# SayanoAI/Comfy-RVC

Measured on AMD Instinct MI355X. Metric: audio-sec/wall-sec (xRT), 40k_v2 end-to-end VC, higher is better.
Workload: dtype f32; 1 GPU; Full VC 40k_v2 (HuBERT -> RMVPE -> SynthesizerTrnMs768NSFsid), 30 s 16 kHz clips, 12 per GPU per step (3 in flight), vc_single host array in -> int16 host array out (BASELINE.json configs[2]); clips_in_flight_per_gpu=3, weights=procedural (comfy-rvc_amd/synthetic.py), noise=device generator, seeded per clip, parallelism=clip-per-GPU x1 (3 lanes each), one RCCL gather of the step's int16 waveforms

## Files before the change

### comfy-rvc_amd/_lib.py

```python
import ctypes as C
import os

_HERE = os.path.dirname(os.path.abspath(__file__))
LIB_PATH = os.environ.get("RVC_HIP_LIB") or os.path.join(_HERE, "csrc", "librvc_hip.so")


class RvcHipError(RuntimeError):
    pass


def _load():
    if not os.path.isfile(LIB_PATH):
        raise RvcHipError(
            f"{LIB_PATH} is missing: build it with `python -c 'import __graft_entry__ as g; g.build()'` "
            "(or `make -C comfy-rvc_amd/csrc`).  There is no CPU fallback.")
    return C.CDLL(LIB_PATH)


lib = _load()

c_void_p, c_int, c_int64, c_float, c_char_p = C.c_void_p, C.c_int, C.c_int64, C.c_float, C.c_char_p
P = C.POINTER


# ... 140 lines not shown
    "rvc_declick": (c_int, [c_void_p, c_void_p, c_int64, c_int, c_float, c_int, c_int, c_int, c_void_p, c_void_p]),
    "rvc_peak_normalize": (c_int, [c_void_p, c_void_p, c_int64, c_float, c_void_p]),
    "rvc_peak_limit": (c_int, [c_void_p, c_void_p, c_int64, c_float]),
    "rvc_merge_tracks": (c_int, [c_void_p, P(c_void_p), P(c_int64), c_int, c_int, c_void_p, c_int64]),
    "rvc_segment_energy": (c_int, [c_void_p, c_void_p, c_int64, c_int, c_void_p]),
    "rvc_spectrogram_batch": (c_int, [c_void_p, c_void_p, c_void_p, c_int64, c_void_p, c_int, c_int, c_int, c_float, c_int, c_void_p, c_int64]),
    "rvc_mel_filterbank_set": (c_int, [c_void_p, c_int, c_int, c_void_p, c_void_p, c_void_p]),
    "rvc_spec_to_mel_batch": (c_int, [c_void_p, c_void_p, c_void_p, c_int64, c_void_p, c_int, c_int, c_int, c_void_p, c_int64]),
    "rvc_spectrogram_batch_ms": (c_int, [c_void_p, c_void_p, c_void_p, c_int64, c_void_p, c_int, c_int, c_int, c_float, c_int, c_void_p, c_int64]),
    "rvc_multiscale_mel_loss": (c_int, [c_void_p, c_void_p, c_int, P(c_void_p), P(c_int64), P(c_int64), c_int, c_int64, P(C.c_int32), P(C.c_int32), c_int, c_int,
                                        c_void_p]),
    "rvc_hpss": (c_int, [c_void_p, c_void_p, c_int, c_int, c_int, c_void_p, c_void_p, c_int]),
    "rvc_hpss_l1": (c_int, [c_void_p, c_void_p, c_void_p, c_int, c_int, c_int, c_float, c_void_p]),
    "rvc_tsi_terms": (c_int, [c_void_p, c_void_p, c_void_p, c_int, c_int, c_int, c_float, c_void_p]),
    "rvc_op_gemm_split": (c_int, [c_void_p] * 7 + [c_int] * 4 + [c_float, c_int, c_float] + [c_int] * 5),
    "rvc_op_conv2d_split": (c_int, [c_void_p] * 7 + [c_int] * 9),
    "rvc_op_wn_in_gate_split": (c_int, [c_void_p] * 6 + [c_int] * 4),
    "rvc_op_gemm_split_qkv": (c_int, [c_void_p] * 6 + [c_int] * 4),
    "rvc_op_conv1d_s2_split": (c_int, [c_void_p] * 6 + [c_int] * 5),
    "rvc_op_conv1d_split": (c_int, [c_void_p] * 6 + [c_int] * 9),
    "rvc_op_conv1d": (c_int, [c_void_p, c_void_p, c_void_p, c_void_p, c_void_p, c_void_p] + [c_int] * 8 +
                      [c_int, c_float, c_int, c_float, c_int, c_float, c_int]),
    "rvc_op_conv_transpose1d": (c_int, [c_void_p, c_void_p, c_void_p, c_void_p, c_void_p] + [c_int] * 6 + [c_int, c_float, c_int]),
    "rvc_op_conv2d3x3": (c_int, [c_void_p, c_void_p, c_void_p, c_void_p, c_void_p, c_void_p] + [c_int] * 5),
    "rvc_op_conv_transpose2d": (c_int, [c_void_p, c_void_p, c_void_p, c_void_p, c_void_p] + [c_int] * 5),
    "rvc_op_gemm_tn": (c_int, [c_void_p, c_void_p, c_void_p, c_void_p] + [c_int] * 4),
    "rvc_conv1d_plan_create": (c_int, [c_void_p, c_void_p] + [c_int] * 7 + [P(c_void_p)]),
    "rvc_conv1d_plan_run": (c_int, [c_void_p, c_void_p, c_void_p, c_int, c_void_p, c_void_p, c_int, c_float, c_int, c_float]),
    "rvc_conv1d_plan_pair_run": (c_int, [c_void_p, c_void_p, c_void_p, c_void_p, c_int, c_void_p, c_float, c_int]),
    "rvc_conv1d_plan_resblock_run": (c_int, [P(c_void_p), c_void_p, c_void_p, c_int, c_void_p, c_float, c_int, P(c_int), c_void_p, c_void_p, c_void_p]),
# ... 108 lines not shown
```

### comfy-rvc_amd/csrc/conv_x3s.hip

```cpp
#include "conv_x3_dev.h"
#include "ops.h"

namespace rvc {

struct GemmSArgs {
  const unsigned char* Wx; int CoPx;
  const unsigned char* Xs; long long xsTp;
  unsigned wx_bytes, xs_bytes;
  int Co, T, nunits;
  int ktaps, margin;
  int toff[16];
  int groups, co_g, rows_pg, cig_chunks;
  unsigned wg_bytes;
  int tdil, tpad;
  int padw; unsigned padmagic;
  const float* bias; const float* R; long long ldR;
  float* Y; long long ldY;
  unsigned char* Ys; long long ysTp;
  int act; float act_slope; int act_before_res; float out_scale;
  int ksplit; float* slabs; unsigned* tickets;
  int gx, gy;
  int xcd_remap;
  int ymargin;
  int zero_tail;
  int row_fast;
  unsigned char* Vt; long long vtTp;
  int vt_row0, vt_rows;
  const float* gate_g; int gate_h;
  int ydeint;
  int seg2_u, seg2_soff;
};

RVC_PHASE_TABLE_REGISTER;

constexpr int x3s_wgs(int AM, int AN, int RS) { return (AM * AN >= 4 && RS != 3) ? 2 : 3; }
template <int AM, int AN, int RS>
__global__ __launch_bounds__(256, x3s_wgs(AM, AN, RS)) void conv_x3s_kernel(const GemmSArgs p) {
  constexpr int WN = 2, NW = 4;
  constexpr int BM = 64 * AM, BN = 64 * AN;
  constexpr int NPA = BM / 16, NPB = BN / 16, NPW = (NPA + NPB) / NW;
  static_assert((NPA % NW) == 0 && (NPB % NW) == 0, "every wave's i-th piece is of one kind");
  constexpr int aslot = BM * 64, bslot = BN * 64, uslot = aslot + bslot;
  static_assert(RS >= 3 && (RS - 2) * NPW <= 63, "ring");
  extern __shared__ __attribute__((aligned(1024))) unsigned char smem3s[];

  const int tid0 = threadIdx.x;
  int lane = tid0 & 63;
  const int wave = __builtin_amdgcn_readfirstlane(tid0 >> 6);
  const int wm = wave / WN, wn = wave % WN;
  const int li = lane & 31, lh = lane >> 5;
  const unsigned total = gridDim.x;
  const unsigned bid = p.xcd_remap ? xcd_tile(blockIdx.x, total) : blockIdx.x;
  const int S = p.ksplit;
  const int tile = (int)(bid / (unsigned)S), ks = (int)(bid - (unsigned)tile * (unsigned)S);
  const int tile_y = p.row_fast ? tile % p.gy : tile / p.gx, tile_x = p.row_fast ? tile / p.gy : tile - tile_y * p.gx;
  const int grp = tile_y / p.rows_pg;
  const int co0 = (tile_y - grp * p.rows_pg) * BM, n0 = tile_x * BN;
  const int row0 = grp * p.co_g, CoG = p.co_g;
// ... 14 lines not shown
#pragma unroll
        for (int an = 0; an < AN; ++an) {
          const int n = n0 + (wn * AN + an) * 32 + li;
          acc[am][an][r] = buf_load(rrs, (r_pre && m < CoG && n < p.T) ? ((unsigned)(row0 + m) * (unsigned)p.ldR + (unsigned)n) * 4u : kOOB) + bv;
        }
      }
  } else {
#pragma unroll
    for (int am = 0; am < AM; ++am)
#pragma unroll
      for (int an = 0; an < AN; ++an)
#pragma unroll
        for (int r = 0; r < 16; ++r) acc[am][an][r] = 0.f;
  }

  const __amdgpu_buffer_rsrc_t ars = make_rsrc(p.Wx, p.wx_bytes), brs = make_rsrc(p.Xs, p.xs_bytes);
  int voff[NPW], dsto[NPW];
#pragma unroll
  for (int i = 0; i < NPW; ++i) {
    const int pi = wave + NW * i;
    if (i * NW < NPA) {
      constexpr int RBK = BM / 64;
      const int plane = pi / RBK, rb = pi - plane * RBK;
      voff[i] = (plane * p.CoPx + co0 + rb * 64 + lane) * 16;
      dsto[i] = plane * (BM * 16) + rb * 1024;
    } else {
      constexpr int CBK = BN / 64;
      const int pj = pi - NPA, plane = pj / CBK, cb = pj - plane * CBK;
      voff[i] = (int)((plane * p.xsTp + n0 + cb * 64 + lane) * 16);
      dsto[i] = aslot + plane * (BN * 16) + cb * 1024;
    }
  }
  const int KT = p.ktaps;
  const int wstep = p.CoPx * 64, cstep = (int)(p.xsTp * 64);
  int tap = u0 % KT;
  bool seg2 = false;
  const bool arith = KT > 16;
  auto tap_off = [&](int t) { return arith ? t * p.tdil - p.tpad : p.toff[t & 15]; };
  int soff_a = (int)((unsigned)grp * p.wg_bytes) + u0 * wstep, soff_c = (grp * p.cig_chunks + u0 / KT) * cstep, soff_b = soff_c + (p.margin + tap_off(tap)) * 16;
  if (u0 >= p.seg2_u) { seg2 = true; soff_b = p.seg2_soff + (u0 - p.seg2_u) * cstep + p.margin * 16; }
  const int seg2_at = p.seg2_u - u0;
  int slw = 0, uw = 0;
  auto issue = [&]() {
    unsigned char* base = smem3s + slw * uslot;
#pragma unroll
    for (int i = 0; i < NPW; ++i) {
      if (i * NW < NPA) buf_dma(ars, base + dsto[i], voff[i], soff_a);
      else buf_dma(brs, base + dsto[i], voff[i], soff_b);
    }
    ++uw;
    if (uw < U1) {
      soff_a += wstep;
      if (uw == seg2_at) { seg2 = true; soff_b = p.seg2_soff + p.margin * 16; }
      else if (KT > 1 && !seg2) {
        ++tap;
        if (tap == KT) { tap = 0; soff_c += cstep; }
        soff_b = soff_c + (p.margin + tap_off(tap)) * 16;
      } else {
        soff_b += cstep;
      }
    }
    slw = slw + 1 == RS ? 0 : slw + 1;
  };

  const int aoff = lh * (BM * 16) + ((wm * AM) * 32 + li) * 16;
  const int boff = aslot + lh * (BN * 16) + ((wn * AN) * 32 + li) * 16;

#pragma unroll
  for (int i = 0; i < RS - 1; ++i) issue();
  wait_vmcnt<(RS - 2) * NPW>();
#pragma unroll
  for (int am = 0; am < AM; ++am)
#pragma unroll
    for (int an = 0; an < AN; ++an) asm volatile("" : "+v"(acc[am][an]));
  lds_barrier();

  struct Ops { u32x4 ah[AM], al[AM], bh[AN], bl[AN]; };
  Ops o0, o1;
  auto read_ops = [&](Ops& o, int slot_i) {
    const unsigned char* wa = smem3s + slot_i * uslot + aoff;
    const unsigned char* xa = smem3s + slot_i * uslot + boff;
#pragma unroll
    for (int am = 0; am < AM; ++am) { o.ah[am] = *reinterpret_cast<const u32x4*>(wa + am * 512); o.al[am] = *reinterpret_cast<const u32x4*>(wa + BM * 32 + am * 512); }
#pragma unroll
    for (int an = 0; an < AN; ++an) { o.bh[an] = *reinterpret_cast<const u32x4*>(xa + an * 512); o.bl[an] = *reinterpret_cast<const u32x4*>(xa + BN * 32 + an * 512); }
  };
  auto mfmas = [&](const Ops& o) {
#pragma unroll
    for (int am = 0; am < AM; ++am)
#pragma unroll
      for (int an = 0; an < AN; ++an)
        acc[am][an] = __builtin_amdgcn_mfma_f32_32x32x16_bf16(__builtin_bit_cast(bf16x8, o.ah[am]), __builtin_bit_cast(bf16x8, o.bl[an]), acc[am][an], 0, 0, 0);
#pragma unroll
    for (int am = 0; am < AM; ++am)
#pragma unroll
      for (int an = 0; an < AN; ++an)
        acc[am][an] = __builtin_amdgcn_mfma_f32_32x32x16_bf16(__builtin_bit_cast(bf16x8, o.al[am]), __builtin_bit_cast(bf16x8, o.bh[an]), acc[am][an], 0, 0, 0);
#pragma unroll
    for (int am = 0; am < AM; ++am)
#pragma unroll
      for (int an = 0; an < AN; ++an)
        acc[am][an] = __builtin_amdgcn_mfma_f32_32x32x16_bf16(__builtin_bit_cast(bf16x8, o.ah[am]), __builtin_bit_cast(bf16x8, o.bh[an]), acc[am][an], 0, 0, 0);
  };
  int sl = 0;
  auto body = [&](const Ops& cur, Ops& nxt) {
    tm.lap(2);
    wait_vmcnt<(RS - 3) * NPW>();
    tm.lap(3);
    lds_barrier();
    tm.lap(4);
    issue();
    sl = sl + 1 == RS ? 0 : sl + 1;
    read_ops(nxt, sl);
    __builtin_amdgcn_sched_barrier(0);
    mfmas(cur);
    __builtin_amdgcn_sched_barrier(0);
  };
  read_ops(o0, 0);
  tm.lap(1);
  int u = 0;
  for (; u + 1 < U1; u += 2) { body(o0, o1); body(o1, o0); }
  if (u < U1) body(o0, o1);
  tm.lap(2);
  asm volatile("s_waitcnt vmcnt(0)" ::: "memory");
  tm.mark();

  if (S > 1) {
    typedef float f32x4_t __attribute__((ext_vector_type(4)));
    constexpr int QN = AM * AN * 4;
    const unsigned slab_bytes = 256u * QN * 16u;
    const __amdgpu_buffer_rsrc_t srs = make_rsrc(p.slabs, (unsigned)(total) * slab_bytes);
    const unsigned lane_off = ((unsigned)wave * QN * 64u + (unsigned)lane) * 16u;
    {
      const unsigned mine = ((unsigned)tile * (unsigned)S + (unsigned)ks) * slab_bytes + lane_off;
#pragma unroll
      for (int am = 0; am < AM; ++am)
#pragma unroll
        for (int an = 0; an < AN; ++an)
#pragma unroll
          for (int q = 0; q < 4; ++q) {
// ... 320 lines not shown
    const int c = hp * 8 + 2 * j;
    if (c < C) Y[(long long)c * ldY + t] = __uint_as_float(hi[j] << 16) + __uint_as_float(lo[j] << 16);
    if (c + 1 < C) Y[(long long)(c + 1) * ldY + t] = __uint_as_float(hi[j] & 0xffff0000u) + __uint_as_float(lo[j] & 0xffff0000u);
  }
}
void split_image_deint_from_f32(hipStream_t s, const float* X, long long ldX, int C, int T, unsigned char* img, long long tp, int H) {
  hipLaunchKernelGGL(split_image_deint_kernel, dim3((T + 255) / 256, (C + 15) / 16 * 2), dim3(256), 0, s, X, ldX, C, T, img, tp, H);
}
void split_image_deint_to_f32(hipStream_t s, const unsigned char* img, long long tp, int H, int C, int T, float* Y, long long ldY) {
  hipLaunchKernelGGL(unsplit_image_deint_kernel, dim3((T + 255) / 256, (C + 15) / 16 * 2), dim3(256), 0, s, img, tp, H, C, T, Y, ldY);
}
void split_image_to_f32(hipStream_t s, const unsigned char* img, long long tp, int C, int T, float* Y, long long ldY) {
  hipLaunchKernelGGL(unsplit_image_kernel, dim3((T + 255) / 256, (C + 15) / 16 * 2), dim3(256), 0, s, img, tp, C, T, Y, ldY);
}

template <int AM, int AN, int RS>
static void launch_x3s(const GemmSArgs& a, unsigned blocks, hipStream_t s) {
  auto kern = conv_x3s_kernel<AM, AN, RS>;
  constexpr size_t lds = (size_t)RS * (64 * AM + 64 * AN) * 64;
  RVC_ALLOW_BIG_LDS(kern);
  conv_launch(kern, dim3(blocks), dim3(256), lds, s, a);
}
static void x3s_dispatch(const GemmSArgs& a, int AM, int AN, unsigned blocks, hipStream_t s) {
  const bool rs3 = AM == 2 && AN == 2 && blocks >= 768u && a.nunits / a.ksplit >= 64;
  if (AM == 2 && AN == 2) { if (rs3) launch_x3s<2, 2, 3>(a, blocks, s); else launch_x3s<2, 2, 4>(a, blocks, s); }
  else if (AM == 2 && AN == 1) launch_x3s<2, 1, 4>(a, blocks, s);
  else if (AM == 1 && AN == 2) launch_x3s<1, 2, 4>(a, blocks, s);
  else launch_x3s<1, 1, 4>(a, blocks, s);
}

static thread_local int t_force_s = 0, t_force_am = 0, t_force_an = 0;
void conv_x3s_force(int ksplit, int am, int an) { t_force_s = ksplit; t_force_am = am; t_force_an = an; }
static void x3s_plan(int M, long long Nplan, int units, int& AM, int& AN, int& S, int groups = 1) {
  static const int target = exp_int("RVC_X3S_BLK", 440);
  auto tiles = [&](int am, int an) { return (long long)groups * ((M + 64 * am - 1) / (64 * am)) * ((Nplan + 64 * an - 1) / (64 * an)); };
  AM = 2; AN = 2;
  const bool deep = units >= 128 && groups == 1 && tiles(2, 2) >= 256;
  if (!deep && tiles(AM, AN) < target) AN = 1;
  if (!deep && tiles(AM, AN) < target) AM = 1;
  if (groups > 1) AM = 1;
  if ((t_force_am == 1 || t_force_am == 2) && groups == 1) AM = t_force_am;
  if (t_force_an == 1 || t_force_an == 2) AN = t_force_an;
  S = 1;
  const long long nt = tiles(AM, AN);
  static const int min_units = exp_int("RVC_X3S_MINUNITS", 32);
  for (int c : {2, 3, 4, 6, 8, 12, 16}) {
    if (nt * S >= target) break;
    if (units % c == 0 && units / c >= min_units) S = c;
  }
  if (t_force_s > 0) S = (units % t_force_s == 0 && units / t_force_s >= 4) ? t_force_s : 1;
}

bool conv_x3s_eligible(const ConvLayer& L) {
  if (L.Wx_ == nullptr || (L.Ci & 15) != 0 || L.Ci * L.ktaps < 32 || L.tconv_u != 0 || L.up2 != 0) return false;
  if (L.mode == 2) return L.ktaps <= 16;
  if (L.mode != 1 || L.stride != 1 || L.pad > kSplitMargin || (L.k - 1) * L.dil - L.pad > kSplitMargin) return false;
  if (L.groups > 1) return (L.Co & 15) == 0 && (L.CoPx & 63) == 0 && L.CoPx <= 64;
  return L.k <= 16 && L.pad == (L.k - 1) / 2 * L.dil && (L.k & 1) == 1;
}

SplitGeom split_geom_s2(int k, long long Tin) {
  SplitGeom g; g.ktaps = k; g.s2_h = split_s2_h(Tin); g.margin = kSplitMargin; g.padw = 0;
  RVC_REQUIRE(k >= 1 && k <= 16, "split_geom_s2: at most 16 taps");
  for (int t = 0; t < k; ++t) g.toff[t] = (t & 1) * g.s2_h + (t >> 1);
  return g;
// ... 59 lines not shown
    a.gate_h = e.gate_h; a.gate_g = e.gate_g;
  }
  a.vt_row0 = 0x7fffffff;
  if (e.vt_out) {
    RVC_REQUIRE(G == 1 && L.mode == 1 && e.vt_row0 > 0 && (e.vt_row0 & 127) == 0 && e.vt_row0 < L.Co && e.vt_tp >= kSplitMargin + (L.Co - e.vt_row0) && Y == nullptr && !e.R && !s2,
                "conv_x3s_run: the transposed rows are the tail of an image-only k = 1 projection, from a multiple of 128 rows on");
    a.Vt = e.vt_out; a.vtTp = e.vt_tp; a.vt_row0 = e.vt_row0; a.vt_rows = L.Co - e.vt_row0;
  }
  a.padmagic = geom->padw > 0 ? (unsigned)((0x100000000ULL + (unsigned)geom->padw - 1) / (unsigned)geom->padw) : 0u;
  for (int t = 0; t < 16; ++t) a.toff[t] = t < geom->ktaps ? geom->toff[t] : 0;
  a.tdil = L.mode == 1 ? L.dil : 1; a.tpad = L.mode == 1 ? L.pad : 0;
  if (s2) { a.tdil = 1; a.tpad = 0; }
  a.groups = G; a.co_g = L.Co; a.cig_chunks = L.Ci / 16; a.wg_bytes = (unsigned)((double)(L.Ci / 16) * geom->ktaps * 4.0 * (double)L.CoPx * 16.0);
  a.bias = e.bias_override ? e.bias_override : L.bd_; a.R = e.R; a.ldR = e.ldR; a.Y = Y; a.ldY = ldY; a.Ys = e.ys_out; a.ysTp = e.ys_tp;
  a.act = e.act; a.act_slope = e.act_slope; a.act_before_res = e.act_before_res; a.out_scale = e.out_scale;
  int AM, AN, S;
  x3s_plan(L.Co, e.plan_tin > 0 ? e.plan_tin : T, a.nunits, AM, AN, S, G);
  const int BM = 64 * AM, BN = 64 * AN;
  RVC_REQUIRE(L.CoPx % BM == 0, "weight image rows are padded to the tile");
  a.rows_pg = (L.Co + BM - 1) / BM;
  a.gx = (T + BN - 1) / BN; a.gy = a.rows_pg * G; a.ksplit = S;
  a.xcd_remap = x3_xcd_remap();
  const unsigned blocks = (unsigned)((long long)a.gx * a.gy * S);
  if (S > 1) {
    const size_t slab_bytes = (size_t)blocks * BM * BN * 4;
    const size_t tick_bytes = ((size_t)a.gx * a.gy * 4 + 255) & ~(size_t)255;
    static const size_t kTickCap = 64 * 1024;
    RVC_REQUIRE(tick_bytes <= kTickCap, "too many tiles for the ticket array");
    bool fresh = false;
    a.tickets = (unsigned*)stream_scratch_zeroed(s, 7, kTickCap, &fresh);
    a.slabs = (float*)stream_scratch(s, 6, slab_bytes);
  }
  ProfTicket tk = conv_prof_begin(s);
  x3s_dispatch(a, AM, AN, blocks, s);
  if (tk.on) {
    ConvArgsX pa{};
    pa.Ci = L.Ci; pa.Co = L.Co; pa.ktaps = geom->ktaps; pa.kreal = geom->ktaps; pa.dil = L.mode == 1 ? L.dil : 1; pa.stride = s2 ? 2 : 1; pa.Tin = T; pa.Tout = T;
    pa.Wd = geom->padw > 0 ? geom->padw - 2 : 0; pa.ksplit = S;
    pa.R = e.R; pa.X = nullptr;
    const double bytes = 4.0 * ((double)L.Ci * T + (double)L.Co * T * ((Y ? 1.0 : 0.0) + (e.ys_out ? 1.0 : 0.0) + (e.R ? 1.0 : 0.0)) + (double)L.Co * L.Ci * geom->ktaps);
    const int id = AM == 2 ? (AN == 2 ? 3 : 5) : (AN == 2 ? 5 : 6);
    conv_prof_end(tk, s, 2.0 * (double)G * L.Co * T * (L.Ci * geom->ktaps + 16 * L.seg2_chunks), 14 + id, bytes * (G > 1 ? (double)G : 1.0), &pa, (long long)blocks, 4 << 4);
  }
}

void conv_x3s_run_swapped(const ConvLayer& L, int row0, int rows, hipStream_t s, const unsigned char* Xs, long long xsTp, int T, unsigned char* Ys, long long ysTp,
                          float* Yrm, long long ldYrm, const float* Rrm, long long ldRrm) {
  RVC_REQUIRE(L.Wx_ != nullptr && L.mode == 1 && L.k == 1 && L.groups == 1 && (L.Ci & 15) == 0, "conv_x3s_run_swapped: a k = 1 projection with a bf16x3 weight image");
  RVC_REQUIRE(row0 >= 0 && rows > 0 && row0 + rows <= L.Co && (row0 & 15) == 0, "conv_x3s_run_swapped: row range");
  RVC_REQUIRE(Xs != nullptr && xsTp >= kSplitMargin + T + 704 && (Ys != nullptr || Yrm != nullptr) && (!Ys || ysTp >= kSplitMargin + rows), "conv_x3s_run_swapped: images missing or too short");
  RVC_REQUIRE(!Yrm || (ldYrm >= rows && (double)T * (double)ldYrm * 4.0 < 2147483648.0), "conv_x3s_run_swapped: row-major output pitch");
  RVC_REQUIRE(!Rrm || (Yrm && ldRrm >= rows && (double)T * (double)ldRrm * 4.0 < 2147483648.0), "conv_x3s_run_swapped: the residual goes with the row-major output");
  const double xs_bytes = (double)(L.Ci / 16) * 4.0 * (double)xsTp * 16.0, wx_bytes = (double)(L.Ci / 16) * 4.0 * (double)L.CoPx * 16.0;
  RVC_REQUIRE(xs_bytes < 2147483648.0 && wx_bytes < 2147483648.0, "operand image exceeds 32-bit buffer addressing");
  GemmSArgs a{};
  a.Wx = Xs + (size_t)kSplitMargin * 16; a.CoPx = (int)xsTp; a.wx_bytes = (unsigned)xs_bytes - (unsigned)kSplitMargin * 16u;
  a.Xs = reinterpret_cast<const unsigned char*>(L.Wx_) + (size_t)row0 * 16; a.xsTp = L.CoPx; a.xs_bytes = (unsigned)wx_bytes - (unsigned)row0 * 16u;
  a.Co = T; a.T = rows; a.nunits = L.Ci / 16; a.ktaps = 1; a.margin = 0; a.ymargin = kSplitMargin; a.zero_tail = 1; a.seg2_u = 0x7fffffff; a.vt_row0 = 0x7fffffff;
  a.groups = 1; a.co_g = T; a.cig_chunks = L.Ci / 16; a.tdil = 1;
  a.Ys = Ys; a.ysTp = ysTp; a.act = ACT_NONE; a.out_scale = 1.f;
  a.Y = Yrm; a.ldY = ldYrm;
  a.R = Rrm; a.ldR = ldRrm;
  int AM, AN, S;
  x3s_plan(T, rows, a.nunits, AM, AN, S);
  S = 1;
  const int BM = 64 * AM, BN = 64 * AN;
  RVC_REQUIRE((long long)((T + BM - 1) / BM) * BM <= xsTp - kSplitMargin && (long long)row0 + (long long)((rows + BN - 1) / BN) * BN <= L.CoPx, "conv_x3s_run_swapped: a tile would read past an operand image");
  a.rows_pg = (T + BM - 1) / BM; a.gx = (rows + BN - 1) / BN; a.gy = a.rows_pg; a.ksplit = 1;
  a.xcd_remap = x3_xcd_remap();
  const unsigned blocks = (unsigned)((long long)a.gx * a.gy);
  ProfTicket tk = conv_prof_begin(s);
  x3s_dispatch(a, AM, AN, blocks, s);
  if (tk.on) {
    ConvArgsX pa{};
    pa.Ci = L.Ci; pa.Co = rows; pa.ktaps = 1; pa.kreal = 1; pa.dil = 1; pa.stride = 1; pa.Tin = T; pa.Tout = T; pa.ksplit = 1;
    const double bytes = 4.0 * ((double)L.Ci * T + (double)rows * T * (Rrm ? 2.0 : 1.0) + (double)rows * L.Ci);
    const int id = AM == 2 ? (AN == 2 ? 3 : 5) : (AN == 2 ? 5 : 6);
    conv_prof_end(tk, s, 2.0 * (double)rows * T * L.Ci, 14 + id, bytes, &pa, (long long)blocks, 4 << 4);
  }
}

}
```

### comfy-rvc_amd/csrc/rvc_api.hip

```cpp
#include "models.h"
#include "conv_kernels.h"

namespace rvc {
static thread_local std::string g_err;
void set_error(const std::string& msg) { g_err = msg; }
}

using namespace rvc;

struct rvc_ctx { Ctx c; };
static std::mutex g_ctx_mu;
static std::map<int, int> g_ctx_count;
struct rvc_hubert { Hubert* m; rvc_ctx* ctx; };
struct rvc_rmvpe { Rmvpe* m; rvc_ctx* ctx; };
struct rvc_synth { Synth* m; rvc_ctx* ctx; };
struct rvc_conv1d_plan { OwnedConvLayer L; };

#define RVC_TRY try {
#define RVC_CATCH                                                            \
  return 0;                                                                  \
  }                                                                          \
  catch (const std::exception& e) { rvc::set_error(e.what()); return 1; }    \
  catch (...) { rvc::set_error("unknown error"); return 2; }

// ... 718 lines not shown
                      int T, int act, float act_slope, int act_before_res, float out_scale, int ksplit, int am, int an, int k, int dil) {
  RVC_TRY
  RVC_REQUIRE(x && w && (y || ysplit_f32) && Ci > 0 && Co > 0 && T > 0 && k >= 1 && (k & 1) == 1 && dil >= 1, "bad argument");
  hipStream_t s = (hipStream_t)stream;
  OwnedConvLayer L;
  { ConvBuildScope scope(2); conv1d_layer_init(L, w, bias, Co, Ci, k, 1, (k - 1) / 2 * dil, dil, 1); }
  RVC_REQUIRE(conv_x3s_eligible(L), "layer not eligible for the split-resident GEMM (Ci % 16 == 0, Ci k >= 64, Co >= 32, pad <= 64)");
  const long long tp = split_image_tp(T);
  DevBytes xs = image_from_f32(s, x, Ci, T, 0), ys;
  ConvEpilogue e; e.act = act; e.act_slope = act_slope; e.act_before_res = act_before_res; e.out_scale = out_scale; e.R = res; e.ldR = T;
  if (ysplit_f32) { ys.alloc(split_image_bytes(Co, T)); e.ys_out = ys.p; e.ys_tp = tp; }
  { X3sForceScope force(ksplit, am, an); conv_x3s_run(L, s, xs.p, tp, T, y, T, e); }
  if (ysplit_f32) split_image_to_f32(s, ys.p, tp, Co, T, ysplit_f32, T);
  check_launch();
  RVC_HIP_CHECK(hipStreamSynchronize(s));
  RVC_CATCH
}
int rvc_op_gemm_split_swapped(void* stream, const float* x, const float* w, float* yt, int Ci, int Co, int T, int row0, int rows) {
  RVC_TRY
  RVC_REQUIRE(x && w && yt && Ci > 0 && Co > 0 && T > 0 && rows > 0, "bad argument");
  hipStream_t s = (hipStream_t)stream;
  OwnedConvLayer L;
  { ConvBuildScope scope(2); conv1d_layer_init(L, w, nullptr, Co, Ci, 1, 1, 0, 1, 1); }
  const long long tp = split_image_tp(T), vtp = attention_vt_tp(rows);
  const size_t vbytes = attention_vt_bytes(rows, T);
  DevBytes xs = image_from_f32(s, x, Ci, T, 0xff), ys;
  ys.alloc(vbytes);
  RVC_HIP_CHECK(hipMemsetAsync(ys.p, 0xff, vbytes, s));
  conv_x3s_run_swapped(L, row0, rows, s, xs.p, tp, T, ys.p, vtp);
  attention_vt_clear_tail(s, ys.p, rows, T);
// ... 635 lines not shown
```

### comfy-rvc_amd/csrc/rvc_internal.h

```cpp
#pragma once
#include <atomic>
#include <hip/hip_runtime.h>
#include <cstdint>
#include <cstdio>
#include <cstdlib>
#include <cmath>
#include <cstring>
#include <map>
#include <mutex>
#include <string>
#include <vector>
#include <stdexcept>

namespace rvc {

void set_error(const std::string& msg);
struct Error : std::runtime_error { using std::runtime_error::runtime_error; };

#define RVC_HIP_CHECK(expr)                                                                       \
  do {                                                                                            \
    hipError_t _e = (expr);                                                                       \
    if (_e != hipSuccess)                                                                         \
      throw rvc::Error(std::string(#expr) + " failed: " + hipGetErrorString(_e) + " (" + __FILE__ + \
                       ":" + std::to_string(__LINE__) + ")");                                     \
// ... 123 lines not shown
inline long long split_s2_tp(long long Tin) { return (kSplitMargin + 2LL * split_s2_h(Tin) + 704 + 63) & ~63LL; }
inline size_t split_s2_bytes(int C, long long Tin) { return (size_t)(C / 16) * 2 * (size_t)split_s2_tp(Tin) * 32; }
SplitGeom split_geom_s2(int k, long long Tin);
bool conv_x3s_s2_eligible(const ConvLayer& L);
inline int wn_gate_row_order(int p, int H) { const int b = p >> 5, q = p & 31; return q < 16 ? 16 * b + q : H + 16 * b + (q - 16); }
void split_image_deint_from_f32(hipStream_t s, const float* X, long long ldX, int C, int T, unsigned char* img, long long tp, int H);
void split_image_deint_to_f32(hipStream_t s, const unsigned char* img, long long tp, int H, int C, int T, float* Y, long long ldY);
bool conv_x3s_eligible(const ConvLayer& L);
void conv_x3s_run(const ConvLayer& L, hipStream_t s, const unsigned char* Xs, long long xsTp, int T, float* Y, long long ldY, const ConvEpilogue& e,
                  const SplitGeom* geom = nullptr);
void conv_x3s_run_swapped(const ConvLayer& L, int row0, int rows, hipStream_t s, const unsigned char* Xs, long long xsTp, int T, unsigned char* Ys, long long ysTp,
                          float* Yrm = nullptr, long long ldYrm = 0,
                          const float* Rrm = nullptr, long long ldRrm = 0);
void split_image_from_tm(hipStream_t s, const float* x, int C, int T, int M, unsigned char* img, long long tp);
void conv_x3s_force(int ksplit, int am, int an);
void x3_weight_image(const float* w, int Co, int Ci, int k, int CoPx, std::vector<uint16_t>& P);
struct ConvX3dArgs {
  const float* X; const unsigned char* Wx; const float* bias; float* Y;
  int Ci, Co, CoPx, H, Hout, p, k, stride, pad, S; float slope;
};
struct ConvX3dPlan { ConvX3dArgs a; dim3 grid; int units = 1; size_t lds = 0; double flops = 0.0; };
bool conv_x3d_plan(const ConvX3dArgs& a, ConvX3dPlan& p);
void conv_x3d_launch(const ConvX3dPlan& p, hipStream_t s);
struct ConvX3dBwdArgs {
  const float* D; const unsigned char* Wx[3]; const float* Cot; const float* A; float* Y;
  int R, RPx, Ck, Hd, H, p, ostride, off0, nph, S; int nt[3]; int Hj[3]; int tile0[4]; float slope;
};
struct ConvX3dBwdPlan { ConvX3dBwdArgs a; dim3 grid; int units = 1; size_t lds = 0; double flops = 0.0; };
bool conv_x3d_bwd_plan(const ConvX3dBwdArgs& a, ConvX3dBwdPlan& p);
void conv_x3d_bwd_launch(const ConvX3dBwdPlan& p, hipStream_t s);
// ... 121 lines not shown
```

### include/rvc_hip.h

```cpp
#ifndef RVC_HIP_H
#define RVC_HIP_H
#include <stdint.h>

#ifdef __cplusplus
extern "C" {
#endif

typedef struct rvc_ctx rvc_ctx;
typedef struct rvc_hubert rvc_hubert;
typedef struct rvc_rmvpe rvc_rmvpe;
typedef struct rvc_synth rvc_synth;

const char* rvc_last_error(void);
const char* rvc_version(void);

int rvc_ctx_create(int device_id, rvc_ctx** out);
int rvc_ctx_destroy(rvc_ctx* ctx);
int64_t rvc_ctx_workspace_bytes(rvc_ctx* ctx);
int rvc_ctx_set_conv_precision(rvc_ctx* ctx, int mode);

typedef struct rvc_hubert_taps {
  float* conv_stack;
  float* pos_conv;
  float* hidden_0;
// ... 191 lines not shown
int rvc_spectrogram_batch_ms(rvc_ctx* ctx, void* stream, const float* audio_dev, int64_t n_audio, const int64_t* clips_host, int n_clips, int n_fft, int hop,
                             float eps, int clamp, float* out_dev, int64_t pitch);
int rvc_multiscale_mel_loss(rvc_ctx* ctx, void* stream, int K, const float* const* spec_dev, const int64_t* pitch, const int64_t* row_stride, int B, int64_t nf,
                            const int32_t* n_fft, const int32_t* n_mels, int loss, int want_mag, double* out_dev);

int rvc_hpss(void* stream, const float* x_dev, int B, int F, int T, float* h_dev, float* p_dev, int medians);
int rvc_hpss_l1(void* stream, const float* org_dev, const float* gen_dev, int B, int F, int T, float eps, double* sums_dev);
int rvc_tsi_terms(void* stream, const float* org_dev, const float* gen_dev, int B, int F, int T, float eps, double* out_dev);

int rvc_op_conv1d(void* stream, const float* x_dev, const float* w_host, const float* bias_host, const float* res_dev, float* y_dev,
                  int Ci, int Co, int Tin, int k, int stride, int pad, int dil, int groups, int pre_act, float pre_slope, int act,
                  float act_slope, int act_before_res, float out_scale, int accumulate);
int rvc_op_gemm_split(void* stream, const float* x_dev, const float* w_host, const float* bias_host, const float* res_dev, float* y_dev,
                      float* ysplit_f32_dev, int Ci, int Co, int T, int act, float act_slope, int act_before_res, float out_scale, int ksplit,
                      int am, int an, int k, int dil);
int rvc_op_conv1d_split(void* stream, const float* x_dev, const float* w_host, const float* bias_host, const float* res_dev, float* y_dev,
                        int Ci, int Co, int T, int k, int pad, int dil, int groups, int act, int act_before_res);
int rvc_op_conv1d_s2_split(void* stream, const float* x_dev, const float* w_host, const float* bias_host, float* y_dev, float* y_img_f32_dev, int Ci, int Co, int T, int k,
                           int act);
int rvc_op_conv2d_split(void* stream, const float* x_dev, const float* w_host, const float* bias_host, const float* res_dev, float* y_dev,
                        float* ysplit_f32_dev, int Ci, int Co, int H, int W, int act, int act_before_res, int ksplit, int am, int an);
int rvc_op_conv_transpose1d(void* stream, const float* x_dev, const float* w_host, const float* bias_host, float* y_dev, int Ci, int Co,
                            int Tin, int k, int u, int pad, int pre_act, float pre_slope, int accumulate);
int rvc_op_conv2d3x3(void* stream, const float* x_dev, const float* w_host, const float* bias_host, const float* res_dev, float* y_dev,
                     int Ci, int Co, int H, int W, int relu);
int rvc_op_conv_transpose2d(void* stream, const float* x_dev, const float* w_host, const float* bias_host, float* y_dev, int Ci, int Co,
                            int H, int W, int relu);
int rvc_op_gemm_tn(void* stream, const float* a_dev, const float* b_dev, float* y_dev, int M, int N, int K, int batch);
typedef struct rvc_conv1d_plan rvc_conv1d_plan;
int rvc_conv1d_plan_create(const float* w_host, const float* bias_host, int Ci, int Co, int k, int stride, int pad, int dil, int groups,
// ... 79 lines not shown
```

Before: 2397 audio-sec/wall-sec.

## Add wave-private K-split main loop for 64x64 conv_x3s tiles

Adds a WP variant of the bf16 MFMA conv kernel for 64x64 tiles. In it, each of the four waves streams its own interleaved subset of K units into a private two-slot LDS ring and computes the full tile, with no per-step workgroup barrier. The partial accumulators are reduced through LDS at the end. The planner enables this path by default for small-grid or deep-K shapes, and a force hook is exposed to override the choice. The aim is to remove the per-iteration lds_barrier and synchronisation stalls on latency-bound small tiles, at the cost of four times the MFMA work per wave on replicated tiles, a final reduction step, and occupancy capped at 2 workgroups.

Result: no change. 2396 audio-sec/wall-sec (-0.0%).

```diff
diff --git a/comfy-rvc_amd/_lib.py b/comfy-rvc_amd/_lib.py
--- a/comfy-rvc_amd/_lib.py
+++ b/comfy-rvc_amd/_lib.py
@@ -178,6 +178,7 @@
     "rvc_hpss_l1": (c_int, [c_void_p, c_void_p, c_void_p, c_int, c_int, c_int, c_float, c_void_p]),
     "rvc_tsi_terms": (c_int, [c_void_p, c_void_p, c_void_p, c_int, c_int, c_int, c_float, c_void_p]),
     "rvc_op_gemm_split": (c_int, [c_void_p] * 7 + [c_int] * 4 + [c_float, c_int, c_float] + [c_int] * 5),
+    "rvc_op_x3s_force_loop": (c_int, [c_int] * 3),
     "rvc_op_conv2d_split": (c_int, [c_void_p] * 7 + [c_int] * 9),
     "rvc_op_wn_in_gate_split": (c_int, [c_void_p] * 6 + [c_int] * 4),
     "rvc_op_gemm_split_qkv": (c_int, [c_void_p] * 6 + [c_int] * 4),
diff --git a/comfy-rvc_amd/csrc/conv_x3s.hip b/comfy-rvc_amd/csrc/conv_x3s.hip
--- a/comfy-rvc_amd/csrc/conv_x3s.hip
+++ b/comfy-rvc_amd/csrc/conv_x3s.hip
@@ -33,15 +33,15 @@
 
 RVC_PHASE_TABLE_REGISTER;
 
-constexpr int x3s_wgs(int AM, int AN, int RS) { return (AM * AN >= 4 && RS != 3) ? 2 : 3; }
-template <int AM, int AN, int RS>
-__global__ __launch_bounds__(256, x3s_wgs(AM, AN, RS)) void conv_x3s_kernel(const GemmSArgs p) {
+constexpr int x3s_wgs(int AM, int AN, int RS, int WP) { return (WP || (AM * AN >= 4 && RS != 3)) ? 2 : 3; }
+template <int AM, int AN, int RS, int WP = 0>
+__global__ __launch_bounds__(256, x3s_wgs(AM, AN, RS, WP)) void conv_x3s_kernel(const GemmSArgs p) {
   constexpr int WN = 2, NW = 4;
   constexpr int BM = 64 * AM, BN = 64 * AN;
   constexpr int NPA = BM / 16, NPB = BN / 16, NPW = (NPA + NPB) / NW;
   static_assert((NPA % NW) == 0 && (NPB % NW) == 0, "every wave's i-th piece is of one kind");
   constexpr int aslot = BM * 64, bslot = BN * 64, uslot = aslot + bslot;
-  static_assert(RS >= 3 && (RS - 2) * NPW <= 63, "ring");
+  static_assert(WP ? (AM == 1 && AN == 1 && RS == 2) : (RS >= 3 && (RS - 2) * NPW <= 63), "ring");
   extern __shared__ __attribute__((aligned(1024))) unsigned char smem3s[];
 
   const int tid0 = threadIdx.x;
@@ -86,116 +86,220 @@
         for (int r = 0; r < 16; ++r) acc[am][an][r] = 0.f;
   }
 
-  const __amdgpu_buffer_rsrc_t ars = make_rsrc(p.Wx, p.wx_bytes), brs = make_rsrc(p.Xs, p.xs_bytes);
-  int voff[NPW], dsto[NPW];
-#pragma unroll
-  for (int i = 0; i < NPW; ++i) {
-    const int pi = wave + NW * i;
-    if (i * NW < NPA) {
-      constexpr int RBK = BM / 64;
-      const int plane = pi / RBK, rb = pi - plane * RBK;
-      voff[i] = (plane * p.CoPx + co0 + rb * 64 + lane) * 16;
-      dsto[i] = plane * (BM * 16) + rb * 1024;
-    } else {
-      constexpr int CBK = BN / 64;
-      const int pj = pi - NPA, plane = pj / CBK, cb = pj - plane * CBK;
-      voff[i] = (int)((plane * p.xsTp + n0 + cb * 64 + lane) * 16);
-      dsto[i] = aslot + plane * (BN * 16) + cb * 1024;
-    }
-  }
-  const int KT = p.ktaps;
-  const int wstep = p.CoPx * 64, cstep = (int)(p.xsTp * 64);
-  int tap = u0 % KT;
-  bool seg2 = false;
-  const bool arith = KT > 16;
-  auto tap_off = [&](int t) { return arith ? t * p.tdil - p.tpad : p.toff[t & 15]; };
-  int soff_a = (int)((unsigned)grp * p.wg_bytes) + u0 * wstep, soff_c = (grp * p.cig_chunks + u0 / KT) * cstep, soff_b = soff_c + (p.margin + tap_off(tap)) * 16;
-  if (u0 >= p.seg2_u) { seg2 = true; soff_b = p.seg2_soff + (u0 - p.seg2_u) * cstep + p.margin * 16; }
-  const int seg2_at = p.seg2_u - u0;
-  int slw = 0, uw = 0;
-  auto issue = [&]() {
-    unsigned char* base = smem3s + slw * uslot;
-#pragma unroll
-    for (int i = 0; i < NPW; ++i) {
-      if (i * NW < NPA) buf_dma(ars, base + dsto[i], voff[i], soff_a);
-      else buf_dma(brs, base + dsto[i], voff[i], soff_b);
-    }
-    ++uw;
-    if (uw < U1) {
-      soff_a += wstep;
-      if (uw == seg2_at) { seg2 = true; soff_b = p.seg2_soff + p.margin * 16; }
-      else if (KT > 1 && !seg2) {
-        ++tap;
-        if (tap == KT) { tap = 0; soff_c += cstep; }
-        soff_b = soff_c + (p.margin + tap_off(tap)) * 16;
-      } else {
-        soff_b += cstep;
-      }
-    }
-    slw = slw + 1 == RS ? 0 : slw + 1;
-  };
-
-  const int aoff = lh * (BM * 16) + ((wm * AM) * 32 + li) * 16;
-  const int boff = aslot + lh * (BN * 16) + ((wn * AN) * 32 + li) * 16;
-
-#pragma unroll
-  for (int i = 0; i < RS - 1; ++i) issue();
-  wait_vmcnt<(RS - 2) * NPW>();
-#pragma unroll
-  for (int am = 0; am < AM; ++am)
-#pragma unroll
-    for (int an = 0; an < AN; ++an) asm volatile("" : "+v"(acc[am][an]));
-  lds_barrier();
-
-  struct Ops { u32x4 ah[AM], al[AM], bh[AN], bl[AN]; };
-  Ops o0, o1;
-  auto read_ops = [&](Ops& o, int slot_i) {
-    const unsigned char* wa = smem3s + slot_i * uslot + aoff;
-    const unsigned char* xa = smem3s + slot_i * uslot + boff;
-#pragma unroll
-    for (int am = 0; am < AM; ++am) { o.ah[am] = *reinterpret_cast<const u32x4*>(wa + am * 512); o.al[am] = *reinterpret_cast<const u32x4*>(wa + BM * 32 + am * 512); }
-#pragma unroll
-    for (int an = 0; an < AN; ++an) { o.bh[an] = *reinterpret_cast<const u32x4*>(xa + an * 512); o.bl[an] = *reinterpret_cast<const u32x4*>(xa + BN * 32 + an * 512); }
-  };
-  auto mfmas = [&](const Ops& o) {
-#pragma unroll
-    for (int am = 0; am < AM; ++am)
-#pragma unroll
-      for (int an = 0; an < AN; ++an)
-        acc[am][an] = __builtin_amdgcn_mfma_f32_32x32x16_bf16(__builtin_bit_cast(bf16x8, o.ah[am]), __builtin_bit_cast(bf16x8, o.bl[an]), acc[am][an], 0, 0, 0);
-#pragma unroll
-    for (int am = 0; am < AM; ++am)
-#pragma unroll
-      for (int an = 0; an < AN; ++an)
-        acc[am][an] = __builtin_amdgcn_mfma_f32_32x32x16_bf16(__builtin_bit_cast(bf16x8, o.al[am]), __builtin_bit_cast(bf16x8, o.bh[an]), acc[am][an], 0, 0, 0);
-#pragma unroll
-    for (int am = 0; am < AM; ++am)
-#pragma unroll
-      for (int an = 0; an < AN; ++an)
-        acc[am][an] = __builtin_amdgcn_mfma_f32_32x32x16_bf16(__builtin_bit_cast(bf16x8, o.ah[am]), __builtin_bit_cast(bf16x8, o.bh[an]), acc[am][an], 0, 0, 0);
-  };
-  int sl = 0;
-  auto body = [&](const Ops& cur, Ops& nxt) {
+  if constexpr (WP) {
+    const __amdgpu_buffer_rsrc_t ars = make_rsrc(p.Wx, p.wx_bytes), brs = make_rsrc(p.Xs, p.xs_bytes);
+    const int va = (co0 + lane) * 16, vb = (n0 + lane) * 16;
+    const int apl = p.CoPx * 16, bpl = (int)(p.xsTp * 16);
+    const int KT = p.ktaps;
+    const int wstep = p.CoPx * 64, cstep = (int)(p.xsTp * 64);
+    const bool arith = KT > 16;
+    auto tap_off = [&](int t) { return arith ? t * p.tdil - p.tpad : p.toff[t & 15]; };
+    const int nmine = U1 > wave ? (U1 - wave + 3) >> 2 : 0;
+    int g = u0 + wave;
+    int tap = g % KT;
+    int soff_a = (int)((unsigned)grp * p.wg_bytes) + g * wstep, soff_c = (grp * p.cig_chunks + g / KT) * cstep;
+    unsigned char* const ring = smem3s + wave * (RS * uslot);
+    auto b_off = [&]() { return g >= p.seg2_u ? p.seg2_soff + (g - p.seg2_u) * cstep + p.margin * 16 : soff_c + (p.margin + tap_off(tap)) * 16; };
+    int soff_b = b_off();
+    auto issue = [&](int slot) {
+      unsigned char* base = ring + slot * uslot;
+#pragma unroll
+      for (int pl = 0; pl < 4; ++pl) buf_dma(ars, base + pl * 1024, va, soff_a + pl * apl);
+#pragma unroll
+      for (int pl = 0; pl < 4; ++pl) buf_dma(brs, base + aslot + pl * 1024, vb, soff_b + pl * bpl);
+      g += NW; soff_a += NW * wstep;
+      if (KT == 1) soff_c += NW * cstep;
+      else { tap += NW; while (tap >= KT) { tap -= KT; soff_c += cstep; } }
+      soff_b = b_off();
+    };
+    struct Ops { u32x4 ah[2], al[2], bh[2], bl[2]; };
+    const int roff = lh * 1024 + li * 16;
+    auto read_ops = [&](Ops& o, int slot) {
+      const unsigned char* wa = ring + slot * uslot + roff;
+      const unsigned char* xa = wa + aslot;
+#pragma unroll
+      for (int i = 0; i < 2; ++i) { o.ah[i] = *reinterpret_cast<const u32x4*>(wa + i * 512); o.al[i] = *reinterpret_cast<const u32x4*>(wa + 2048 + i * 512); }
+#pragma unroll
+      for (int i = 0; i < 2; ++i) { o.bh[i] = *reinterpret_cast<const u32x4*>(xa + i * 512); o.bl[i] = *reinterpret_cast<const u32x4*>(xa + 2048 + i * 512); }
+    };
+    f32x16 pw[2][2];
+    if (nmine > 0) issue(0);
+    if (nmine > 1) issue(1);
+    if (nmine > 1) wait_vmcnt<8>(); else wait_vmcnt<0>();
+    asm volatile("" : "+v"(acc[0][0]));
+#pragma unroll
+    for (int am = 0; am < 2; ++am)
+#pragma unroll
+      for (int an = 0; an < 2; ++an)
+#pragma unroll
+        for (int r = 0; r < 16; ++r) pw[am][an][r] = 0.f;
+    Ops o0, o1;
+    if (nmine > 0) read_ops(o0, 0);
+    tm.lap(1);
+    auto mfma4 = [&](const u32x4 (&a)[2], const u32x4 (&b)[2]) {
+#pragma unroll
+      for (int am = 0; am < 2; ++am)
+#pragma unroll
+        for (int an = 0; an < 2; ++an)
+          pw[am][an] = __builtin_amdgcn_mfma_f32_32x32x16_bf16(__builtin_bit_cast(bf16x8, a[am]), __builtin_bit_cast(bf16x8, b[an]), pw[am][an], 0, 0, 0);
+    };
+    auto body = [&](int j, const Ops& cur, Ops& nxt, int slot) {
+      asm volatile("s_waitcnt lgkmcnt(0)" ::: "memory");
+      __builtin_amdgcn_sched_barrier(0);
+      if (j + 2 < nmine) issue(slot);
+      __builtin_amdgcn_sched_barrier(0);
+      mfma4(cur.ah, cur.bl);
+      mfma4(cur.al, cur.bh);
+      __builtin_amdgcn_sched_barrier(0);
+      if (j + 1 < nmine) {
+        tm.lap(2);
+        if (j + 2 < nmine) wait_vmcnt<8>(); else wait_vmcnt<0>();
+        tm.lap(3);
+        read_ops(nxt, slot ^ 1);
+      }
+      __builtin_amdgcn_sched_barrier(0);
+      mfma4(cur.ah, cur.bh);
+      __builtin_amdgcn_sched_barrier(0);
+    };
+    int j = 0;
+    for (; j + 1 < nmine; j += 2) { body(j, o0, o1, 0); body(j + 1, o1, o0, 1); }
+    if (j < nmine) body(j, o0, o1, 0);
     tm.lap(2);
-    wait_vmcnt<(RS - 3) * NPW>();
-    tm.lap(3);
+    asm volatile("s_waitcnt vmcnt(0)" ::: "memory");
+    lds_barrier();
+    typedef float f32x4r __attribute__((ext_vector_type(4)));
+#pragma unroll
+    for (int am = 0; am < 2; ++am)
+#pragma unroll
+      for (int an = 0; an < 2; ++an)
+#pragma unroll
+        for (int q = 0; q < 4; ++q)
+          *reinterpret_cast<f32x4r*>(smem3s + ((am * 2 + an) * NW + wave) * 4096 + q * 1024 + lane * 16) =
+              f32x4r{pw[am][an][4 * q], pw[am][an][4 * q + 1], pw[am][an][4 * q + 2], pw[am][an][4 * q + 3]};
+    lds_barrier();
+#pragma unroll
+    for (int w = 0; w < NW; ++w)
+#pragma unroll
+      for (int q = 0; q < 4; ++q) {
+        const f32x4r v = *reinterpret_cast<const f32x4r*>(smem3s + (wave * NW + w) * 4096 + q * 1024 + lane * 16);
+#pragma unroll
+        for (int e = 0; e < 4; ++e) acc[0][0][4 * q + e] += v[e];
+      }
     lds_barrier();
     tm.lap(4);
-    issue();
-    sl = sl + 1 == RS ? 0 : sl + 1;
-    read_ops(nxt, sl);
-    __builtin_amdgcn_sched_barrier(0);
-    mfmas(cur);
-    __builtin_amdgcn_sched_barrier(0);
-  };
-  read_ops(o0, 0);
-  tm.lap(1);
-  int u = 0;
-  for (; u + 1 < U1; u += 2) { body(o0, o1); body(o1, o0); }
-  if (u < U1) body(o0, o1);
-  tm.lap(2);
-  asm volatile("s_waitcnt vmcnt(0)" ::: "memory");
-  tm.mark();
+  } else {
+    const __amdgpu_buffer_rsrc_t ars = make_rsrc(p.Wx, p.wx_bytes), brs = make_rsrc(p.Xs, p.xs_bytes);
+    int voff[NPW], dsto[NPW];
+  #pragma unroll
+    for (int i = 0; i < NPW; ++i) {
+      const int pi = wave + NW * i;
+      if (i * NW < NPA) {
+        constexpr int RBK = BM / 64;
+        const int plane = pi / RBK, rb = pi - plane * RBK;
+        voff[i] = (plane * p.CoPx + co0 + rb * 64 + lane) * 16;
+        dsto[i] = plane * (BM * 16) + rb * 1024;
+      } else {
+        constexpr int CBK = BN / 64;
+        const int pj = pi - NPA, plane = pj / CBK, cb = pj - plane * CBK;
+        voff[i] = (int)((plane * p.xsTp + n0 + cb * 64 + lane) * 16);
+        dsto[i] = aslot + plane * (BN * 16) + cb * 1024;
+      }
+    }
+    const int KT = p.ktaps;
+    const int wstep = p.CoPx * 64, cstep = (int)(p.xsTp * 64);
+    int tap = u0 % KT;
+    bool seg2 = false;
+    const bool arith = KT > 16;
+    auto tap_off = [&](int t) { return arith ? t * p.tdil - p.tpad : p.toff[t & 15]; };
+    int soff_a = (int)((unsigned)grp * p.wg_bytes) + u0 * wstep, soff_c = (grp * p.cig_chunks + u0 / KT) * cstep, soff_b = soff_c + (p.margin + tap_off(tap)) * 16;
+    if (u0 >= p.seg2_u) { seg2 = true; soff_b = p.seg2_soff + (u0 - p.seg2_u) * cstep + p.margin * 16; }
+    const int seg2_at = p.seg2_u - u0;
+    int slw = 0, uw = 0;
+    auto issue = [&]() {
+      unsigned char* base = smem3s + slw * uslot;
+  #pragma unroll
+      for (int i = 0; i < NPW; ++i) {
+        if (i * NW < NPA) buf_dma(ars, base + dsto[i], voff[i], soff_a);
+        else buf_dma(brs, base + dsto[i], voff[i], soff_b);
+      }
+      ++uw;
+      if (uw < U1) {
+        soff_a += wstep;
+        if (uw == seg2_at) { seg2 = true; soff_b = p.seg2_soff + p.margin * 16; }
+        else if (KT > 1 && !seg2) {
+          ++tap;
+          if (tap == KT) { tap = 0; soff_c += cstep; }
+          soff_b = soff_c + (p.margin + tap_off(tap)) * 16;
+        } else {
+          soff_b += cstep;
+        }
+      }
+      slw = slw + 1 == RS ? 0 : slw + 1;
+    };
+
+    const int aoff = lh * (BM * 16) + ((wm * AM) * 32 + li) * 16;
+    const int boff = aslot + lh * (BN * 16) + ((wn * AN) * 32 + li) * 16;
+
+  #pragma unroll
+    for (int i = 0; i < RS - 1; ++i) issue();
+    wait_vmcnt<(RS - 2) * NPW>();
+  #pragma unroll
+    for (int am = 0; am < AM; ++am)
+  #pragma unroll
+      for (int an = 0; an < AN; ++an) asm volatile("" : "+v"(acc[am][an]));
+    lds_barrier();
+
+    struct Ops { u32x4 ah[AM], al[AM], bh[AN], bl[AN]; };
+    Ops o0, o1;
+    auto read_ops = [&](Ops& o, int slot_i) {
+      const unsigned char* wa = smem3s + slot_i * uslot + aoff;
+      const unsigned char* xa = smem3s + slot_i * uslot + boff;
+  #pragma unroll
+      for (int am = 0; am < AM; ++am) { o.ah[am] = *reinterpret_cast<const u32x4*>(wa + am * 512); o.al[am] = *reinterpret_cast<const u32x4*>(wa + BM * 32 + am * 512); }
+  #pragma unroll
+      for (int an = 0; an < AN; ++an) { o.bh[an] = *reinterpret_cast<const u32x4*>(xa + an * 512); o.bl[an] = *reinterpret_cast<const u32x4*>(xa + BN * 32 + an * 512); }
+    };
+    auto mfmas = [&](const Ops& o) {
+  #pragma unroll
+      for (int am = 0; am < AM; ++am)
+  #pragma unroll
+        for (int an = 0; an < AN; ++an)
+          acc[am][an] = __builtin_amdgcn_mfma_f32_32x32x16_bf16(__builtin_bit_cast(bf16x8, o.ah[am]), __builtin_bit_cast(bf16x8, o.bl[an]), acc[am][an], 0, 0, 0);
+  #pragma unroll
+      for (int am = 0; am < AM; ++am)
+  #pragma unroll
+        for (int an = 0; an < AN; ++an)
+          acc[am][an] = __builtin_amdgcn_mfma_f32_32x32x16_bf16(__builtin_bit_cast(bf16x8, o.al[am]), __builtin_bit_cast(bf16x8, o.bh[an]), acc[am][an], 0, 0, 0);
+  #pragma unroll
+      for (int am = 0; am < AM; ++am)
+  #pragma unroll
+        for (int an = 0; an < AN; ++an)
+          acc[am][an] = __builtin_amdgcn_mfma_f32_32x32x16_bf16(__builtin_bit_cast(bf16x8, o.ah[am]), __builtin_bit_cast(bf16x8, o.bh[an]), acc[am][an], 0, 0, 0);
+    };
+    int sl = 0;
+    auto body = [&](const Ops& cur, Ops& nxt) {
+      tm.lap(2);
+      wait_vmcnt<(RS - 3) * NPW>();
+      tm.lap(3);
+      lds_barrier();
+      tm.lap(4);
+      issue();
+      sl = sl + 1 == RS ? 0 : sl + 1;
+      read_ops(nxt, sl);
+      __builtin_amdgcn_sched_barrier(0);
+      mfmas(cur);
+      __builtin_amdgcn_sched_barrier(0);
+    };
+    read_ops(o0, 0);
+    tm.lap(1);
+    int u = 0;
+    for (; u + 1 < U1; u += 2) { body(o0, o1); body(o1, o0); }
+    if (u < U1) body(o0, o1);
+    tm.lap(2);
+    asm volatile("s_waitcnt vmcnt(0)" ::: "memory");
+    tm.mark();
+
+  }
 
   if (S > 1) {
     typedef float f32x4_t __attribute__((ext_vector_type(4)));
@@ -546,24 +650,28 @@
   hipLaunchKernelGGL(unsplit_image_kernel, dim3((T + 255) / 256, (C + 15) / 16 * 2), dim3(256), 0, s, img, tp, C, T, Y, ldY);
 }
 
-template <int AM, int AN, int RS>
+template <int AM, int AN, int RS, int WP = 0>
 static void launch_x3s(const GemmSArgs& a, unsigned blocks, hipStream_t s) {
-  auto kern = conv_x3s_kernel<AM, AN, RS>;
-  constexpr size_t lds = (size_t)RS * (64 * AM + 64 * AN) * 64;
+  auto kern = conv_x3s_kernel<AM, AN, RS, WP>;
+  constexpr size_t lds = WP ? (size_t)4 * RS * 8192 : (size_t)RS * (64 * AM + 64 * AN) * 64;
   RVC_ALLOW_BIG_LDS(kern);
   conv_launch(kern, dim3(blocks), dim3(256), lds, s, a);
 }
-static void x3s_dispatch(const GemmSArgs& a, int AM, int AN, unsigned blocks, hipStream_t s) {
+static void x3s_dispatch(const GemmSArgs& a, int AM, int AN, bool wp, unsigned blocks, hipStream_t s) {
   const bool rs3 = AM == 2 && AN == 2 && blocks >= 768u && a.nunits / a.ksplit >= 64;
+  RVC_REQUIRE(!wp || (AM == 1 && AN == 1), "conv_x3s: the wave-private loop belongs to the 64 x 64 tile");
   if (AM == 2 && AN == 2) { if (rs3) launch_x3s<2, 2, 3>(a, blocks, s); else launch_x3s<2, 2, 4>(a, blocks, s); }
   else if (AM == 2 && AN == 1) launch_x3s<2, 1, 4>(a, blocks, s);
   else if (AM == 1 && AN == 2) launch_x3s<1, 2, 4>(a, blocks, s);
+  else if (wp) launch_x3s<1, 1, 2, 1>(a, blocks, s);
   else launch_x3s<1, 1, 4>(a, blocks, s);
 }
 
 static thread_local int t_force_s = 0, t_force_am = 0, t_force_an = 0;
+static thread_local int t_hold_am = 0, t_hold_an = 0, t_hold_loop = 0;
 void conv_x3s_force(int ksplit, int am, int an) { t_force_s = ksplit; t_force_am = am; t_force_an = an; }
-static void x3s_plan(int M, long long Nplan, int units, int& AM, int& AN, int& S, int groups = 1) {
+void conv_x3s_force_loop(int am, int an, int loop) { t_hold_am = am; t_hold_an = an; t_hold_loop = loop; }
+static void x3s_plan(int M, long long Nplan, int units, int& AM, int& AN, int& S, bool& WP, int groups = 1) {
   static const int target = exp_int("RVC_X3S_BLK", 440);
   auto tiles = [&](int am, int an) { return (long long)groups * ((M + 64 * am - 1) / (64 * am)) * ((Nplan + 64 * an - 1) / (64 * an)); };
   AM = 2; AN = 2;
@@ -571,8 +679,9 @@
   if (!deep && tiles(AM, AN) < target) AN = 1;
   if (!deep && tiles(AM, AN) < target) AM = 1;
   if (groups > 1) AM = 1;
-  if ((t_force_am == 1 || t_force_am == 2) && groups == 1) AM = t_force_am;
-  if (t_force_an == 1 || t_force_an == 2) AN = t_force_an;
+  const int fam = t_force_am ? t_force_am : t_hold_am, fan = t_force_an ? t_force_an : t_hold_an;
+  if ((fam == 1 || fam == 2) && groups == 1) AM = fam;
+  if (fan == 1 || fan == 2) AN = fan;
   S = 1;
   const long long nt = tiles(AM, AN);
   static const int min_units = exp_int("RVC_X3S_MINUNITS", 32);
@@ -581,6 +690,13 @@
     if (units % c == 0 && units / c >= min_units) S = c;
   }
   if (t_force_s > 0) S = (units % t_force_s == 0 && units / t_force_s >= 4) ? t_force_s : 1;
+  static const int wp_mode = exp_int("RVC_X3S_WP", 1);
+  const long long wgs = nt * S;
+  const int u1 = units / S;
+  const bool wp_class = (wgs <= 512 && u1 >= 18) || (u1 >= 96 && (wgs + 511) / 512 == (wgs + 767) / 768);
+  WP = AM == 1 && AN == 1 && (wp_mode == 2 || (wp_mode == 1 && wp_class));
+  if (t_hold_loop == 1) WP = false;
+  if (t_hold_loop == 2) WP = true;
 }
 
 bool conv_x3s_eligible(const ConvLayer& L) {
@@ -670,8 +786,8 @@
   a.groups = G; a.co_g = L.Co; a.cig_chunks = L.Ci / 16; a.wg_bytes = (unsigned)((double)(L.Ci / 16) * geom->ktaps * 4.0 * (double)L.CoPx * 16.0);
   a.bias = e.bias_override ? e.bias_override : L.bd_; a.R = e.R; a.ldR = e.ldR; a.Y = Y; a.ldY = ldY; a.Ys = e.ys_out; a.ysTp = e.ys_tp;
   a.act = e.act; a.act_slope = e.act_slope; a.act_before_res = e.act_before_res; a.out_scale = e.out_scale;
-  int AM, AN, S;
-  x3s_plan(L.Co, e.plan_tin > 0 ? e.plan_tin : T, a.nunits, AM, AN, S, G);
+  int AM, AN, S; bool WP;
+  x3s_plan(L.Co, e.plan_tin > 0 ? e.plan_tin : T, a.nunits, AM, AN, S, WP, G);
   const int BM = 64 * AM, BN = 64 * AN;
   RVC_REQUIRE(L.CoPx % BM == 0, "weight image rows are padded to the tile");
   a.rows_pg = (L.Co + BM - 1) / BM;
@@ -688,7 +804,7 @@
     a.slabs = (float*)stream_scratch(s, 6, slab_bytes);
   }
   ProfTicket tk = conv_prof_begin(s);
-  x3s_dispatch(a, AM, AN, blocks, s);
+  x3s_dispatch(a, AM, AN, WP, blocks, s);
   if (tk.on) {
     ConvArgsX pa{};
     pa.Ci = L.Ci; pa.Co = L.Co; pa.ktaps = geom->ktaps; pa.kreal = geom->ktaps; pa.dil = L.mode == 1 ? L.dil : 1; pa.stride = s2 ? 2 : 1; pa.Tin = T; pa.Tout = T;
@@ -717,8 +833,8 @@
   a.Ys = Ys; a.ysTp = ysTp; a.act = ACT_NONE; a.out_scale = 1.f;
   a.Y = Yrm; a.ldY = ldYrm;
   a.R = Rrm; a.ldR = ldRrm;
-  int AM, AN, S;
-  x3s_plan(T, rows, a.nunits, AM, AN, S);
+  int AM, AN, S; bool WP;
+  x3s_plan(T, rows, a.nunits, AM, AN, S, WP);
   S = 1;
   const int BM = 64 * AM, BN = 64 * AN;
   RVC_REQUIRE((long long)((T + BM - 1) / BM) * BM <= xsTp - kSplitMargin && (long long)row0 + (long long)((rows + BN - 1) / BN) * BN <= L.CoPx, "conv_x3s_run_swapped: a tile would read past an operand image");
@@ -726,7 +842,7 @@
   a.xcd_remap = x3_xcd_remap();
   const unsigned blocks = (unsigned)((long long)a.gx * a.gy);
   ProfTicket tk = conv_prof_begin(s);
-  x3s_dispatch(a, AM, AN, blocks, s);
+  x3s_dispatch(a, AM, AN, WP, blocks, s);
   if (tk.on) {
     ConvArgsX pa{};
     pa.Ci = L.Ci; pa.Co = rows; pa.ktaps = 1; pa.kreal = 1; pa.dil = 1; pa.stride = 1; pa.Tin = T; pa.Tout = T; pa.ksplit = 1;
diff --git a/comfy-rvc_amd/csrc/rvc_api.hip b/comfy-rvc_amd/csrc/rvc_api.hip
--- a/comfy-rvc_amd/csrc/rvc_api.hip
+++ b/comfy-rvc_amd/csrc/rvc_api.hip
@@ -756,6 +756,12 @@
   if (ysplit_f32) split_image_to_f32(s, ys.p, tp, Co, T, ysplit_f32, T);
   check_launch();
   RVC_HIP_CHECK(hipStreamSynchronize(s));
+  RVC_CATCH
+}
+int rvc_op_x3s_force_loop(int am, int an, int loop) {
+  RVC_TRY
+  RVC_REQUIRE(am >= 0 && am <= 2 && an >= 0 && an <= 2 && loop >= 0 && loop <= 2, "tile factors 0 .. 2, loop 0 (planner), 1 (ring) or 2 (wave-private)");
+  conv_x3s_force_loop(am, an, loop);
   RVC_CATCH
 }
 int rvc_op_gemm_split_swapped(void* stream, const float* x, const float* w, float* yt, int Ci, int Co, int T, int row0, int rows) {
diff --git a/comfy-rvc_amd/csrc/rvc_internal.h b/comfy-rvc_amd/csrc/rvc_internal.h
--- a/comfy-rvc_amd/csrc/rvc_internal.h
+++ b/comfy-rvc_amd/csrc/rvc_internal.h
@@ -161,6 +161,7 @@
                           const float* Rrm = nullptr, long long ldRrm = 0);
 void split_image_from_tm(hipStream_t s, const float* x, int C, int T, int M, unsigned char* img, long long tp);
 void conv_x3s_force(int ksplit, int am, int an);
+void conv_x3s_force_loop(int am, int an, int loop);
 void x3_weight_image(const float* w, int Co, int Ci, int k, int CoPx, std::vector<uint16_t>& P);
 struct ConvX3dArgs {
   const float* X; const unsigned char* Wx; const float* bias; float* Y;
diff --git a/include/rvc_hip.h b/include/rvc_hip.h
--- a/include/rvc_hip.h
+++ b/include/rvc_hip.h
@@ -229,6 +229,7 @@
 int rvc_op_gemm_split(void* stream, const float* x_dev, const float* w_host, const float* bias_host, const float* res_dev, float* y_dev,
                       float* ysplit_f32_dev, int Ci, int Co, int T, int act, float act_slope, int act_before_res, float out_scale, int ksplit,
                       int am, int an, int k, int dil);
+int rvc_op_x3s_force_loop(int am, int an, int loop);
 int rvc_op_conv1d_split(void* stream, const float* x_dev, const float* w_host, const float* bias_host, const float* res_dev, float* y_dev,
                         int Ci, int Co, int T, int k, int pad, int dil, int groups, int act, int act_before_res);
 int rvc_op_conv1d_s2_split(void* stream, const float* x_dev, const float* w_host, const float* bias_host, float* y_dev, float* y_img_f32_dev, int Ci, int Co, int T, int k,
```
